# TimingSpace/MVOScaleRecovery

Measured on AMD Instinct MI355X. Metric: frames/sec scale-recovery, KITTI-00 flow (~2k feats/frame), 1/2/4/8 GPU, higher is better.
Workload: dtype f64

## Files before the change

### mvoscalerecovery_amd/csrc/mvosr_kernels.hip

```cpp
#include <hip/hip_runtime.h>
#include <math.h>
#include <stdint.h>
#include <stdlib.h>
#include <string.h>

#include "../../include/mvosr.h"
#include "mvosr_device.hpp"
#include "mvosr_host.hpp"
#include "mvosr_npsum.hpp"

namespace mvosr {

#ifdef MVOSR_STAMPS
#define MVOSR_STAMP(i) do { if (threadIdx.x == 0 && stamps) stamps[i] = __builtin_amdgcn_s_memtime(); } while (0)
#define MVOSR_STAMP_DECL unsigned long long stamps[12] = {0,0,0,0,0,0,0,0,0,0,0,0};
#define MVOSR_STAMP_ARG , unsigned long long *stamps = nullptr
#define MVOSR_STAMP_PASS , stamps
#define MVOSR_RSTAMP(i) do { if (stamps) stamps[i] = __builtin_amdgcn_s_memtime(); } while (0)
#else
#define MVOSR_RSTAMP(i) do {} while (0)
#define MVOSR_STAMP(i) do {} while (0)
#define MVOSR_STAMP_DECL
#define MVOSR_STAMP_ARG
#define MVOSR_STAMP_PASS
// ... 567 lines not shown
            if (base + k * B + tid < t2_count) mark_triangle(base / B + k, tc.q[k].a, tc.q[k].b, tc.q[k].c);
        }
        if (more) tc = tn;
    }
    bad |= bad_in;
    int sn = singular | (near << 16);
    block_sum4i<WAVES>(npitch, ntv, sn, bad, s.red + R_SEL_CNT * 2 * WAVES);
    singular = sn & 0xFFFF;
    r.near = sn >> 16;
    MVOSR_STAMP(5);
    r.height_level = MODE == MODE_HOT ? hl / 3.0 : hl;
    r.n_steep = (int)hcnt;
    r.n_pitch = npitch; r.n_tri_valid = ntv; r.singular = singular; r.bad = bad;
    return r;
}

struct RoadResult {
    double height;
    int status;
    int n_sel, n_kept, n_modes, mode_left, mode_right;
    double mean, std, skew, median;
};

__device__ __forceinline__ bool dropped_by_single(double y, int bin, const Bits192 &single, int first_single) {
    bool d = false;
#pragma unroll
    for (int dk = -1; dk <= 1; ++dk) {
        const int k = bin + dk;
        const bool is_single = (k >= 0) && (k < kBins) && single.test_lane(max(k, 0));
        const double r = bin_edge(k + 1);
        const double lo = r - 0.1;
        const bool in = (k == first_single) ? (y >= lo && y <= r) : (y > lo && y <= r);
        d |= is_single && in;
    }
    return d;
}

#ifdef MVOSR_ROAD_EXACT_COUNT
__device__ unsigned long long g_road_exact_count[3];
#endif
constexpr int kRoadRC = 20;
constexpr int kRoadSub = 4;
constexpr int kRoadWaves = 4;
constexpr int kTrash = 175;
constexpr int kStPending = -1;
constexpr int kStRedo = -2;
static_assert(kStRedo == MVOSR_ST_REDO, "include/mvosr.h");
constexpr int kMaxVoteRows = 32765;

struct RoadArgs {
    mvosr_params P;
    const int64_t *off;
    const int32_t *cnt;
    const double *y;
    double *scratch;
    const double *height_level;
    mvosr_outputs o;
    int64_t first_frame, n_frames;
    int pending_only;
    int32_t *level_redo;
    const int32_t *list;
    int wide;
    const uint8_t *listed_mask = nullptr;
};

__device__ __forceinline__ int bin_of_table(double y, const double2 *edges) {
    if (!(y >= 0.0 && y <= bin_edge(kBins))) return -1;
    int k = min((int)(y * 10.0), kBins - 1);
    const double2 e = edges[k];
    k += (k < kBins - 1 && y >= e.y) ? 1 : 0;
    k -= (y < e.x) ? 1 : 0;
    return k;
}

template <int RC, int WW = 1>
__device__ __forceinline__ RoadResult road_wave(int *hist, int *comb, uint8_t *nearflag, const double2 *edges,
                                                const double *yv_all, double *scratch,
                                                int Mall, double height_level, const mvosr_params &P, int32_t *g_hist, bool exact_stats,
                                                int part_lo, int part_hi, double *part, int *np_stack MVOSR_STAMP_ARG) {
    static_assert(RC <= 32 && kRoadSub == 4, "32-bit row masks; one int4 per bin");
    const int lane = lane_id();
    RoadResult R;
    R.height = nan(""); R.status = MVOSR_ST_MODE; R.n_sel = Mall; R.n_kept = 0; R.n_modes = 0; R.mode_left = -1; R.mode_right = -1;
    R.mean = R.std = R.skew = R.median = nan("");
    if (Mall == 0) { R.status = MVOSR_ST_NO_FLAT; return R; }
    const double *yv = yv_all + (part_hi > part_lo ? part_lo : 0);
    const int M = part_hi - part_lo;
    if (WW == 1 || wave_id() == 0) {
        int4 z; z.x = z.y = z.z = z.w = 0;
#pragma unroll
        for (int c = 0; c < 3; ++c) { const int b = lane + 64 * c; if (b < 176) reinterpret_cast<int4 *>(hist)[b] = z; }
    }
    if constexpr (WW > 1) __syncthreads();
    const double y0 = yv_all[0];
    const double sh = (y0 - y0 == 0.0) ? y0 : 0.0;
    int *hsub = hist + (lane & (kRoadSub - 1));

    const int nfull = M / kWave;
// ... 3 lines not shown
    unsigned pk[(RC + 3) / 4];
    constexpr int kG = 4;
#pragma unroll
    for (int k0 = 0; k0 < RC; k0 += kG) {
        double yg[kG];
#pragma unroll
        for (int j = 0; j < kG && k0 + j < RC; ++j) yg[j] = yv[max(min((k0 + j) * kWave + lane, M - 1), 0)];
#pragma unroll
        for (int j = 0; j < kG && k0 + j < RC; ++j) {
            const int k = k0 + j;
            const double y = yg[j];
            const bool vk = (valid >> k) & 1u;
            const bool inr = vk && (y >= 0.0) && (y <= bin_edge(kBins));
            const int g = inr ? min((int)(y * 10.0), kBins - 1) : 0;
            const double2 e = edges[g];
            int bin = g + ((g < kBins - 1 && y >= e.y) ? 1 : 0) - ((y < e.x) ? 1 : 0);
            bin = inr ? bin : kTrash;
            atomicAdd(&hsub[4 * bin], 1);
            const double d = vk ? y - sh : 0.0;
            s1 += d;
            s2 = __builtin_fma(d, d, s2);
            pk[k >> 2] = (k & 3) ? (pk[k >> 2] | ((unsigned)bin << (8 * (k & 3)))) : (unsigned)bin;
        }
        __builtin_amdgcn_sched_barrier(0);
    }
    constexpr int kLongUnroll = 2;
    for (int i0 = RC * kWave + lane; i0 < M; i0 += kLongUnroll * kWave) {
        double yl[kLongUnroll];
#pragma unroll
        for (int j = 0; j < kLongUnroll; ++j) yl[j] = yv[max(min(i0 + j * kWave, M - 1), 0)];
#pragma unroll
        for (int j = 0; j < kLongUnroll; ++j) {
            if (i0 + j * kWave >= M) continue;
            const int bin = bin_of_table(yl[j], edges);
            if (bin >= 0) atomicAdd(&hsub[4 * bin], 1);
            const double d = yl[j] - sh;
            s1 += d;
            s2 = __builtin_fma(d, d, s2);
        }
    }
    MVOSR_RSTAMP(2);
    if constexpr (WW > 1) __syncthreads();
    int hraw[3], hz[3];
    Bits192 single, modes, mins;
    int mx = 0, mn = 0x7fffffff;
#pragma unroll
    for (int c = 0; c < 3; ++c) {
        const int b = lane + 64 * c;
        int h = 0;
        if (b < kBins) { const int4 q = reinterpret_cast<const int4 *>(hist)[b]; h = (q.x + q.y) + (q.z + q.w); }
        if (b < 176) comb[b] = h;
        hraw[c] = h;
        hz[c] = (hraw[c] == 1) ? 0 : hraw[c];
        single.w[c] = __ballot(b < kBins && hraw[c] == 1);
        mx = max(mx, hz[c]);
        if (b < kBins) mn = min(mn, hz[c]);
    }
    mx = wave_max(mx);
    mn = wave_min(mn);
    if (g_hist && (WW == 1 || wave_id() == 0)) {
#pragma unroll
        for (int c = 0; c < 3; ++c) { const int b = lane + 64 * c; if (b < kBins) { g_hist[b] = hraw[c]; g_hist[kBins + b] = hz[c]; } }
    }
    MVOSR_RSTAMP(3);
    const int first_single = single.lowest_from(0);
    Bits192 near;
    near.w[0] = single.w[0] | (single.w[0] << 1) | (single.w[0] >> 1) | (single.w[1] << 63);
    near.w[1] = single.w[1] | (single.w[1] << 1) | (single.w[1] >> 1) | (single.w[0] >> 63) | (single.w[2] << 63);
    near.w[2] = single.w[2] | (single.w[2] << 1) | (single.w[2] >> 1) | (single.w[1] >> 63);
#pragma unroll
    for (int c = 0; c < 3; ++c) { const int b = lane + 64 * c; if (b < 176) nearflag[b] = (b < kBins) ? (uint8_t)((near.w[c] >> lane) & 1ull) : 0; }
    const bool have_modes = mx > P.mode_min;

    double t1 = 0.0, t2 = 0.0;
    int nd = 0;
    {
        unsigned sus = 0u;
#pragma unroll
        for (int k = 0; k < RC; ++k) sus |= (nearflag[(pk[k >> 2] >> (8 * (k & 3))) & 0xFFu] ? 1u : 0u) << k;
        while (sus) {
            const int k = __ffs(sus) - 1;
            sus &= sus - 1u;
            const double y = yv[k * kWave + lane];
            if (dropped_by_single(y, bin_of_table(y, edges), single, first_single)) {
                const double d = y - sh;
                t1 += d;
                t2 = __builtin_fma(d, d, t2);
                ++nd;
            }
        }
    }
    for (int i0 = RC * kWave + lane; i0 < M; i0 += kLongUnroll * kWave) {
        double yl[kLongUnroll];
#pragma unroll
        for (int j = 0; j < kLongUnroll; ++j) yl[j] = yv[max(min(i0 + j * kWave, M - 1), 0)];
#pragma unroll
        for (int j = 0; j < kLongUnroll; ++j) {
            if (i0 + j * kWave >= M) continue;
            const double y = yl[j];
            const int bin = bin_of_table(y, edges);
            if (bin >= 0 && nearflag[bin] && dropped_by_single(y, bin, single, first_single)) {
                const double d = y - sh;
                t1 += d;
                t2 = __builtin_fma(d, d, t2);
                ++nd;
            }
        }
    }
    double S1 = wave_sum(s1 - t1), S2 = wave_sum(s2 - t2), Q = wave_sum(s2);
    nd = wave_sum(nd);
    if constexpr (WW > 1) {
        if (lane == 0) { part[4 * wave_id()] = S1; part[4 * wave_id() + 1] = S2; part[4 * wave_id() + 2] = Q; part[4 * wave_id() + 3] = (double)nd; }
        __syncthreads();
        S1 = 0.0; S2 = 0.0; Q = 0.0;
        double ndd = 0.0;
#pragma unroll
        for (int i = 0; i < WW; ++i) { S1 += part[4 * i]; S2 += part[4 * i + 1]; Q += part[4 * i + 2]; ndd += part[4 * i + 3]; }
        nd = (int)ndd;
    }
    MVOSR_RSTAMP(4);
    const int nkept = Mall - nd;
    const double cntd = (double)nkept;
    R.n_kept = nkept;

    auto pack_kept = [&]() {
        int nlist = 0;
#pragma unroll 1
        for (int i0 = 0; i0 < Mall; i0 += kWave) {
            const int i = i0 + lane;
            bool keep = false;
            double y = 0.0;
            if (i < Mall) {
                y = yv_all[i];
                const int bin = bin_of_table(y, edges);
                keep = !(bin >= 0 && nearflag[bin] && dropped_by_single(y, bin, single, first_single));
            }
            const unsigned long long m = __ballot(keep);
            if (keep) scratch[nlist + __popcll(m & ((1ull << lane) - 1ull))] = y;
            nlist += __popcll(m);
        }
        return nlist;
    };

    if (!have_modes) {
        if constexpr (WW > 1) { if (wave_id() != 0) return R; }
        if (nkept == 0) { R.height = height_level; R.status = MVOSR_ST_LEVEL; return R; }
        pack_kept();
        __threadfence_block();
        const int klo = (nkept - 1) >> 1, khi = nkept >> 1;
        double mlo = 0.0, mhi = 0.0;
        int flo = 0, fhi = 0;
        for (int i = lane; i < nkept; i += kWave) {
            const double yi = scratch[i];
            int rank = 0;
            for (int j = 0; j < nkept; ++j) {
                const double yj = scratch[j];
                rank += (yj < yi) || (yj == yi && j < i);
            }
            if (rank == klo) { mlo = yi; flo = 1; }
            if (rank == khi) { mhi = yi; fhi = 1; }
        }
        const unsigned long long blo = __ballot(flo), bhi = __ballot(fhi);
        mlo = readlane_d(mlo, (int)__ffsll((long long)blo) - 1);
        mhi = readlane_d(mhi, (int)__ffsll((long long)bhi) - 1);
        R.median = (klo == khi) ? mlo : (mlo + mhi) / 2.0;
        R.height = R.median; R.status = MVOSR_ST_MEDIAN;
        return R;
    }
    if constexpr (WW > 1) { if (wave_id() != 0) return R; }
// ... 32 lines not shown
    const double right = bin_edge(ir + 1);
    const double m1 = S1 / cntd;
    const double mean = sh + m1;
    const double var = S2 / cntd - m1 * m1;
    double mean_o = mean;
    double sd = sqrt(var);
    {
        const double thr = fabs(P.skew_threshold);
        const double N = (double)Mall;
        const double g = 0x1p-52 * (2.0 * (double)((Mall + kWave - 1) / kWave) + 64.0 + N / (double)kNpBufSize);
        const double a2 = Q / cntd, r = sqrt(a2), rho = sqrt(N / cntd), Mg = fabs(sh) + r;
        const double rms = sqrt(mean * mean + var);
        const double margin = fabs((mean - mode / 10.0) - P.skew_threshold * sd);
        const double bound_two_pass = 1e-11 * (rms + sd) + 1e-22 * rms * rms / sd;
        const double bound = bound_two_pass
                           + g * ((Mg + rho * r) + fabs(mode / 10.0) + (1.0 + thr) * sd + (1.0 + thr) * (a2 * (6.0 + 2.0 * rho) + g * Mg * Mg) / sd);
#ifdef MVOSR_ROAD_EXACT_COUNT
        if (lane == 0) {
            atomicAdd(&g_road_exact_count[0], 1ull);
            if (!(margin > bound_two_pass)) atomicAdd(&g_road_exact_count[1], 1ull);
            if (!(margin > bound)) atomicAdd(&g_road_exact_count[2], 1ull);
        }
#endif
        if (!(margin > bound) || exact_stats) {
            const int nl = pack_kept();
            __threadfence_block();
            mean_o = np_pairwise_sum_cold(scratch, nl, 0.0, 0, np_stack) / (double)nl;
            sd = sqrt(np_pairwise_sum_cold(scratch, nl, mean_o, 1, np_stack) / (double)nl);
        }
    }
    const double skew = (mean_o - mode / 10.0) / sd;
    R.mean = mean_o; R.std = sd; R.skew = skew;
    if (skew > P.skew_threshold) { R.height = right; R.status = MVOSR_ST_RIGHT; }
    else { R.height = mode / 10.0; R.status = MVOSR_ST_MODE; }
    return R;
}

constexpr int kRoadOcc = 6;
template <bool LIST, int WW = 1>
__global__ __launch_bounds__(kRoadWaves *kWave, (LIST ? 1 : kRoadOcc)) void road_model_kernel(const RoadArgs a) {
    static_assert(kRoadRC >= 16 && kRoadRC <= 32, "the row masks are 32 bits");
    static_assert(WW == 1 || (WW == kRoadWaves && !LIST), "wide variant: the whole workgroup on one frame");
    __shared__ __attribute__((aligned(16))) int hist_all[kRoadWaves][kRoadSub * 176];
    __shared__ int comb_all[kRoadWaves][176];
    __shared__ uint8_t near_all[kRoadWaves][176];
    __shared__ double2 edges[kBins + 1];
    __shared__ double part[4 * kRoadWaves];
    __shared__ __attribute__((aligned(8))) int np_stack_all[kRoadWaves][kNpStackInts];
    for (int k = threadIdx.x; k < kBins; k += kRoadWaves * kWave) { double2 e; e.x = bin_edge(k); e.y = bin_edge(k + 1); edges[k] = e; }
    __syncthreads();
    const int64_t slot = WW > 1 ? (int64_t)blockIdx.x : (int64_t)blockIdx.x * kRoadWaves + wave_id();
    auto one_frame = [&](const int64_t f) {
    if (a.pending_only && a.o.status[f] != kStPending) return;
    MVOSR_STAMP_DECL
    MVOSR_RSTAMP(0);
    const int M = a.cnt[f];
    const int64_t off = a.off[f];
    const double hl = a.height_level ? a.height_level[f] : nan("");
    MVOSR_RSTAMP(1);
    int *h0 = hist_all[WW > 1 ? 0 : wave_id()];
    int32_t *gh = a.o.hist ? a.o.hist + f * 2 * kBins : nullptr;
    const bool ex = a.o.stats != nullptr;
    int lo = 0, hi = M;
    if constexpr (WW > 1) {
        const int q = ((M + WW * kWave - 1) / (WW * kWave)) * kWave;
        lo = min(M, wave_id() * q);
        hi = min(M, lo + q);
    }
    const int Mp = hi - lo;
#define MVOSR_ROAD_CALL(RC_) road_wave<RC_, WW>(h0, comb_all[wave_id()], near_all[wave_id()], edges, a.y + off, a.scratch + off, M, hl, a.P, gh, ex, lo, hi, part, np_stack_all[wave_id()] MVOSR_STAMP_PASS)
    const RoadResult R = (Mp <= 4 * kWave) ? MVOSR_ROAD_CALL(4)
                       : (Mp <= 8 * kWave) ? MVOSR_ROAD_CALL(8)
                       : (Mp <= 12 * kWave) ? MVOSR_ROAD_CALL(12)
                       : (Mp <= 16 * kWave) ? MVOSR_ROAD_CALL(16)
                                            : MVOSR_ROAD_CALL(kRoadRC);
#undef MVOSR_ROAD_CALL
    MVOSR_RSTAMP(6);
#ifdef MVOSR_STAMPS
    if (lane_id() == 0 && a.o.hist) { unsigned long long *d = reinterpret_cast<unsigned long long *>(a.o.hist + f * 2 * kBins) + 16; for (int i = 0; i < 8; ++i) d[i] = stamps[i]; }
#endif
    if (WW > 1 && wave_id() != 0) return;
    if (R.status == MVOSR_ST_LEVEL && a.level_redo) {
        if (lane_id() == 0) {
            if (!(a.listed_mask && a.listed_mask[f])) a.level_redo[1 + atomicAdd(a.level_redo, 1)] = (int32_t)f;
            a.o.status[f] = kStRedo;
        }
        return;
    }
    if (lane_id() == 0) {
        double height = nan(""), raw = nan("");
        if (R.status == MVOSR_ST_NO_FLAT) raw = a.P.absolute_reference / hl;
        else if (R.status <= MVOSR_ST_LEVEL) { height = R.height; raw = a.P.absolute_reference / height; }
        a.o.raw_scale[f] = raw; a.o.height[f] = height; a.o.status[f] = R.status;
        if (!a.pending_only && a.o.height_level) a.o.height_level[f] = hl;
        if (a.o.counts) {
            int32_t *c = a.o.counts + f * MVOSR_N_COUNTS;
            if (!a.pending_only) { c[MVOSR_CNT_VALID] = M; c[MVOSR_CNT_TRI_PITCH] = 0; c[MVOSR_CNT_TRI_VALID] = 0; }
            c[MVOSR_CNT_SELECTED] = R.n_sel; c[MVOSR_CNT_KEPT] = R.n_kept; c[MVOSR_CNT_MODES] = R.n_modes;
            c[MVOSR_CNT_MODE_LEFT] = R.mode_left; c[MVOSR_CNT_MODE_RIGHT] = R.mode_right;
        }
        if (a.o.stats) { double *st = a.o.stats + 4 * f; st[0] = R.mean; st[1] = R.std; st[2] = R.skew; st[3] = R.median; }
    }
    };
    if constexpr (LIST) {
        const int64_t n_todo = (int64_t)a.list[0];
        for (int64_t it = slot; it < n_todo; it += (int64_t)gridDim.x * kRoadWaves) one_frame((int64_t)a.list[1 + it]);
    } else {
        if (slot < a.n_frames) one_frame(a.first_frame + slot);
    }
}

struct KArgs {
    mvosr_params P;
    mvosr_batch b;
    mvosr_outputs o;
    PitchTest pt;
    int64_t first_frame;
    const double *height_level_in;
    int32_t *redo;
    int redo_pass;
    double *ysel;
    int32_t *nsel;
    const int32_t *cls_list;
    const int32_t *cls_cnt;
};

__device__ __forceinline__ void write_counts(const KArgs &a, int64_t f, int nvalid, int npitch, int ntv, const RoadResult &R) {
    if (!a.o.counts) return;
    int32_t *c = a.o.counts + f * MVOSR_N_COUNTS;
// ... 1042 lines not shown
    if (b->max_feat > variant_capacity(waves, sc))
        return set_error(MVOSR_ERR_TOO_LARGE, "%d features exceed what %d wavefronts per frame handle (%d)", b->max_feat, waves,
                         variant_capacity(waves, sc));
    if ((int64_t)2 * b->max_feat > (int64_t)64 * kWave * waves)
        return set_error(MVOSR_ERR_TOO_LARGE, "%d features give more triangles than %d wavefronts sweep", b->max_feat, waves);
    return MVOSR_OK;
}

__global__ __launch_bounds__(256) void append_mask_kernel(const uint8_t *mask, const int32_t *status, int64_t first, int64_t n, int32_t *redo) {
    const int64_t k = (int64_t)blockIdx.x * blockDim.x + threadIdx.x;
    if (k >= n) return;
    const int64_t f = first + k;
    if (mask[f] && (!status || status[f] == kStPending)) redo[1 + atomicAdd(redo, 1)] = (int32_t)f;
}
static int launch_append_mask(mvosr_ctx *ctx, const KArgs &ka, int64_t nl, bool check_status) {
    if (!ka.b.exact_mask) return MVOSR_OK;
    hipLaunchKernelGGL(append_mask_kernel, dim3((unsigned)((nl + 255) / 256)), dim3(256), 0, ctx_stream(ctx), ka.b.exact_mask,
                       check_status ? ka.o.status : (const int32_t *)nullptr, ka.first_frame, nl, ka.redo);
    return check_launch("append_mask_kernel");
}

constexpr int kRedoGrid = 512;
constexpr int kModeExactList = 3;
static inline KArgs &kargs_of(KArgs &a) { return a; }
static inline KArgs &kargs_of(DenseArgs &a) { return a.k; }

static thread_local bool g_hot_only = false;

template <class Args>
static int launch_modes(mvosr_ctx *ctx, void (*k_hot)(const Args), void (*k_exact)(const Args), void (*k_full)(const Args),
                        Args args, int64_t nl, int threads, size_t lds, int mode, const char *name, size_t lds_hot = 0,
                        int threads_hot = 0) {
    int rc;
    if (lds_hot == 0) lds_hot = lds;
    if (threads_hot == 0) threads_hot = threads;
    kargs_of(args).redo_pass = 0;
    if (mode == MODE_FULL) {
        if ((rc = prepare_kernel(k_full, lds))) return rc;
        hipLaunchKernelGGL(k_full, dim3((unsigned)nl), dim3(threads), lds, ctx_stream(ctx), args);
        return check_launch(name);
    }
    if ((rc = prepare_kernel(k_exact, lds))) return rc;
    if (mode == kModeExactList) {
        kargs_of(args).redo_pass = 1;
        const unsigned grid = (unsigned)(nl < (int64_t)kRedoGrid ? nl : (int64_t)kRedoGrid);
        hipLaunchKernelGGL(k_exact, dim3(grid), dim3(threads), lds, ctx_stream(ctx), args);
        return check_launch(name);
    }
    if (mode == MODE_EXACT) {
        hipLaunchKernelGGL(k_exact, dim3((unsigned)nl), dim3(threads), lds, ctx_stream(ctx), args);
        return check_launch(name);
    }
    if ((rc = prepare_kernel(k_hot, lds_hot))) return rc;
    const hipError_t e = hipMemsetAsync(kargs_of(args).redo, 0, sizeof(int32_t), ctx_stream(ctx));
    if (e != hipSuccess) return set_hip_error("hipMemsetAsync(redo list)", e);
    hipLaunchKernelGGL(k_hot, dim3((unsigned)nl), dim3(threads_hot), lds_hot, ctx_stream(ctx), args);
    if ((rc = check_launch(name))) return rc;
    if (!g_hot_only && (rc = launch_append_mask(ctx, kargs_of(args), nl, true))) return rc;
    return MVOSR_OK;
}

template <int WAVES, int SC>
static int launch_scale(mvosr_ctx *ctx, const KArgs &ka, int64_t nl, int mode) {
    const size_t lds = lds_plan(ka.b.max_feat, WAVES).total;
    int rc = check_fit(&ka.b, WAVES, SC, lds);
    if (rc) return rc;
    return launch_modes<KArgs>(ctx, scale_frames_kernel<WAVES, SC, MODE_HOT>, scale_frames_kernel<WAVES, SC, MODE_EXACT>,
                               scale_frames_kernel<WAVES, SC, MODE_FULL>, ka, nl, WAVES * kWave, lds, mode, "scale_frames_kernel");
}

template <int WAVES, int SC>
static int launch_vote(mvosr_ctx *ctx, const KArgs &ka, int64_t nl) {
    const size_t lds = lds_plan(ka.b.max_feat, WAVES).total;
    int rc = check_fit(&ka.b, WAVES, SC, lds);
    if (rc) return rc;
    if ((rc = prepare_kernel(outlier_vote_kernel<WAVES, SC>, lds))) return rc;
    hipLaunchKernelGGL((outlier_vote_kernel<WAVES, SC>), dim3((unsigned)nl), dim3(WAVES * kWave), lds, ctx_stream(ctx), ka);
    return check_launch("outlier_vote_kernel");
// ... 22 lines not shown
    }
    if (vote_only) {
        if ((rc = prepare_kernel(outlier_vote_dense_kernel<DW>, lds))) return rc;
        hipLaunchKernelGGL((outlier_vote_dense_kernel<DW>), dim3((unsigned)nl), dim3(DW * kWave), lds, ctx_stream(ctx), da);
        return check_launch("outlier_vote_dense_kernel");
    }
    if (tiled)
        return launch_modes<DenseArgs>(ctx, scale_frames_tiled_kernel<kTiledWaves>, scale_frames_dense_feat_kernel<DW, MODE_EXACT>,
                                       scale_frames_dense_feat_kernel<DW, MODE_FULL>, da, nl, DW * kWave, lds, mode,
                                       "scale_frames_tiled_kernel", tiled_plan(ka.b.max_feat, kTiledWaves).total, kTiledWaves * kWave);
    if (ka.b.tri2_ids == MVOSR_TRI2_FEATURES)
        return launch_modes<DenseArgs>(ctx, scale_frames_dense_feat_kernel<DW, MODE_HOT>, scale_frames_dense_feat_kernel<DW, MODE_EXACT>,
                                       scale_frames_dense_feat_kernel<DW, MODE_FULL>, da, nl, DW * kWave, lds, mode,
                                       "scale_frames_dense_feat_kernel");
    return launch_modes<DenseArgs>(ctx, scale_frames_dense_kernel<DW, MODE_HOT>, scale_frames_dense_kernel<DW, MODE_EXACT>,
                                   scale_frames_dense_kernel<DW, MODE_FULL>, da, nl, DW * kWave, lds, mode, "scale_frames_dense_kernel");
}

static int launch_scale_dense(mvosr_ctx *ctx, const KArgs &ka, int64_t nl, int mode, bool vote_only) {
    if (ka.b.max_feat > 65535) return set_error(MVOSR_ERR_TOO_LARGE, "more than 65535 features per frame");
    return launch_scale_dense_w<kDenseWaves>(ctx, ka, nl, mode, vote_only);
}

static int launch_road(mvosr_ctx *ctx, const RoadArgs &ra, hipStream_t stream) {
    if (ra.n_frames <= 0) return MVOSR_OK;
    if (ra.wide && !ra.list) {
        hipLaunchKernelGGL((road_model_kernel<false, kRoadWaves>), dim3((unsigned)ra.n_frames), dim3(kRoadWaves * kWave), 0, stream, ra);
        return check_launch("road_model_kernel (wide)");
    }
    const unsigned blocks = ra.list ? 64u : (unsigned)((ra.n_frames + kRoadWaves - 1) / kRoadWaves);
    if (ra.list) hipLaunchKernelGGL(road_model_kernel<true>, dim3(blocks), dim3(kRoadWaves * kWave), 0, stream, ra);
    else hipLaunchKernelGGL(road_model_kernel<false>, dim3(blocks), dim3(kRoadWaves * kWave), 0, stream, ra);
    return check_launch("road_model_kernel");
}

#define MVOSR_DISPATCH(FN, ...)                                                             \
    do {                                                                                    \
        const int n_ = ka.b.max_feat;                                                       \
        switch (waves) {                                                                    \
            case 1: return FN<1, 8>(__VA_ARGS__);                                           \
            case 4: return (n_ <= variant_capacity(4, 4)) ? FN<4, 4>(__VA_ARGS__) : FN<4, 8>(__VA_ARGS__);     \
            case 16: return (n_ <= variant_capacity(16, 4)) ? FN<16, 4>(__VA_ARGS__) : FN<16, 8>(__VA_ARGS__); \
            default: return (n_ <= variant_capacity(8, 4)) ? FN<8, 4>(__VA_ARGS__) : FN<8, 8>(__VA_ARGS__);    \
        }                                                                                   \
    } while (0)

static int dispatch_scale(mvosr_ctx *ctx, const KArgs &ka, int waves, int64_t nl, int mode) { MVOSR_DISPATCH(launch_scale, ctx, ka, nl, mode); }
static int dispatch_vote(mvosr_ctx *ctx, const KArgs &ka, int waves, int64_t nl) { MVOSR_DISPATCH(launch_vote, ctx, ka, nl); }

typedef void (*scale_kernel_fn)(const KArgs);
static scale_kernel_fn hot_list_kernel(int waves, int n) {
    switch (waves) {
        case 1: return scale_frames_kernel<1, 8, MODE_HOT, true>;
        case 4: return (n <= variant_capacity(4, 4)) ? scale_frames_kernel<4, 4, MODE_HOT, true> : scale_frames_kernel<4, 8, MODE_HOT, true>;
// ... 14 lines not shown
    scale_kernel_fn fn[3];
    int waves[3];
    size_t lds[3];
    KArgs kc[3];
    for (int c = 0; c < 3; ++c) {
        kc[c] = ka;
        kc[c].b.max_feat = thr[c] < ka.b.max_feat ? thr[c] : ka.b.max_feat;
        const int n = kc[c].b.max_feat;
        waves[c] = pick_waves(0, n);
        lds[c] = lds_plan(n, waves[c]).total;
        fn[c] = hot_list_kernel(waves[c], n);
        const int sc = (n <= variant_capacity(waves[c], 4) && waves[c] != 1) ? 4 : 8;
        if ((rc = check_fit(&kc[c].b, waves[c], sc, lds[c]))) return rc;
        if ((rc = prepare_kernel(fn[c], lds[c]))) return rc;
        int64_t bound = hinted && (int64_t)ka.b.size_hint[c] < nl ? (int64_t)ka.b.size_hint[c] : nl;
        if ((c > 0 && thr[c - 1] >= ka.b.max_feat) || ka.b.min_feat > thr[c]) bound = 0;
        ca.grid[c] = (int)(bound < 0 ? 0 : bound);
        kc[c].cls_list = ca.lists + c * ca.stride;
        kc[c].cls_cnt = hdr + c;
        kc[c].redo_pass = 0;
    }
    if ((e = hipMemsetAsync(hdr, 0, kClassHeader * sizeof(int32_t), ctx_stream(ctx))) != hipSuccess)
        return set_hip_error("hipMemsetAsync(class lists)", e);
    if ((e = hipMemsetAsync(ka.redo, 0, sizeof(int32_t), ctx_stream(ctx))) != hipSuccess)
        return set_hip_error("hipMemsetAsync(redo list)", e);
    const int cb = kClassifyWaves * kWave;
    hipLaunchKernelGGL(classify_frames_kernel, dim3((unsigned)((nl + cb - 1) / cb)), dim3(cb), 0, ctx_stream(ctx), ca);
    if ((rc = check_launch("classify_frames_kernel"))) return rc;
    for (int c = 2; c >= 0; --c) {
        if (ca.grid[c] == 0) continue;
        hipLaunchKernelGGL(fn[c], dim3((unsigned)ca.grid[c]), dim3(waves[c] * kWave), lds[c], ctx_stream(ctx), kc[c]);
        if ((rc = check_launch("scale_frames_kernel (size class)"))) return rc;
    }
    return MVOSR_OK;
}

void set_max_dynamic_lds(int bytes) { g_max_dyn_lds = bytes; }

}

using namespace mvosr;

extern "C" {

void mvosr_default_params(mvosr_params *p, double absolute_reference) {
    if (!p) return;
    const double pitch = -0.5 * 3.141592653589793 / 180.0;
    p->cos_pitch = cos(pitch);
// ... 46 lines not shown
    ra.P = *p; ra.off = b->feat_off; ra.cnt = ka.nsel; ra.y = ka.ysel; ra.scratch = ka.ysel;
    ra.height_level = o->height_level; ra.o = *o; ra.pending_only = 1; ra.level_redo = nullptr; ra.list = nullptr; ra.wide = 0;
    ka.first_frame = first_frame;
    if (b->tri2_ids != MVOSR_TRI2_SURVIVORS && b->tri2_ids != MVOSR_TRI2_FEATURES)
        return set_error(MVOSR_ERR_ARG, "scale_batch: batch.tri2_ids must be MVOSR_TRI2_SURVIVORS or MVOSR_TRI2_FEATURES");
    if (b->tri2_ids == MVOSR_TRI2_FEATURES && !(waves_per_frame == 0 || waves_per_frame == 16))
        return set_error(MVOSR_ERR_ARG, "scale_batch: feature-numbered tri2 runs the gather variant (waves_per_frame 0 or 16)");
    const bool dense = (waves_per_frame == 0 || waves_per_frame == 16) &&
                       (b->max_feat > lds_capacity_features() || b->tri2_ids == MVOSR_TRI2_FEATURES);
    hipEvent_t *pev = (ctx->prof_on && ctx->prof_calls < kProfRing) ? ctx->prof_ev[ctx->prof_calls] : nullptr;
    hipError_t ee = hipSuccess;
    if (pev && (ee = hipEventRecord(pev[0], ctx_stream(ctx))) != hipSuccess) return set_hip_error("hipEventRecord(profile)", ee);
    const bool by_class = mode == MODE_HOT && !dense && waves_per_frame == 0 && n_launch >= kClassMinFrames &&
                          b->max_feat > kClassThr0 &&
                          (b->min_feat <= 0 || pick_waves(0, b->min_feat) != waves);
    const bool standin = b->standin_u != nullptr;
    if (standin) {
        if (!b->standin_keep || !b->standin_rows || !b->standin_cnt || !b->standin_status || !b->tri2_cnt || b->tri2_ids != MVOSR_TRI2_SURVIVORS)
            return set_error(MVOSR_ERR_ARG, "scale_batch: stand-in rows need standin_keep/_rows/_cnt/_status, tri2_cnt and survivor-numbered rows");
        if (dense) return set_error(MVOSR_ERR_TOO_LARGE, "scale_batch: stand-in rows are for frames that fit the LDS-resident kernels");
        if (!(want_masked || mode == MODE_HOT))
            return set_error(MVOSR_ERR_ARG, "scale_batch: stand-in rows need the HOT mode (no stage outputs, no EXACT-for-all)");
    }
    auto road = [&]() {
#ifdef MVOSR_STAMPS
        return MVOSR_OK;
#else
        return launch_road(ctx, ra, ctx_stream(ctx));
#endif
    };
    auto standin_rows = [&](const int32_t *list) {
        return qh_rows_for_list(ctx, b->n_frames, b->feat_off, b->feat_cnt, b->standin_u, b->v, b->standin_keep, b->max_feat, b->tri2_off,
                                b->standin_rows, b->standin_cnt, b->standin_status, list);
    };
    if (want_masked) {
        if (!b->exact_mask) return set_error(MVOSR_ERR_ARG, "scale_batch: MVOSR_WAVES_EXACT_MASKED without batch.exact_mask");
        const hipError_t e0 = hipMemsetAsync(ka.redo, 0, sizeof(int32_t), ctx_stream(ctx));
        if (e0 != hipSuccess) return set_hip_error("hipMemsetAsync(redo list)", e0);
        if ((rc = launch_append_mask(ctx, ka, n_launch, false))) return rc;
        if (standin && (rc = standin_rows(ka.redo))) return rc;
        if ((rc = dense ? launch_scale_dense(ctx, ka, n_launch, kModeExactList, false) : dispatch_scale(ctx, ka, waves, n_launch, kModeExactList))) return rc;
        ra.first_frame = first_frame; ra.n_frames = n_launch; ra.list = ka.redo;
        ra.wide = dense ? 1 : 0;
        return road();
    }
    if (by_class) {
        if ((rc = launch_scale_classes(ctx, ka, n_launch))) return rc;
        if (!hot_only && (rc = launch_append_mask(ctx, ka, n_launch, true))) return rc;
    } else {
        g_hot_only = hot_only;
        rc = dense ? launch_scale_dense(ctx, ka, n_launch, mode, false) : dispatch_scale(ctx, ka, waves, n_launch, mode);
        g_hot_only = false;
        if (rc) return rc;
    }
    if (pev && (ee = hipEventRecord(pev[1], ctx_stream(ctx))) != hipSuccess) return set_hip_error("hipEventRecord(profile)", ee);
    ra.first_frame = first_frame; ra.n_frames = n_launch;
    ra.wide = dense ? 1 : 0;
    if (mode == MODE_HOT) {
        ra.level_redo = ka.redo;
        ra.listed_mask = hot_only ? nullptr : b->exact_mask;
        if ((rc = road())) return rc;
        ra.listed_mask = nullptr;
        if (hot_only) return MVOSR_OK;
        if (standin && (rc = standin_rows(ka.redo))) return rc;
        if ((rc = dense ? launch_scale_dense(ctx, ka, n_launch, kModeExactList, false) : dispatch_scale(ctx, ka, waves, n_launch, kModeExactList))) return rc;
        ra.level_redo = nullptr; ra.list = ka.redo;
        if ((rc = road())) return rc;
    } else if ((rc = road())) {
        return rc;
    }
    if (pev) {
        if ((ee = hipEventRecord(pev[2], ctx_stream(ctx))) != hipSuccess) return set_hip_error("hipEventRecord(profile)", ee);
        ctx->prof_calls++;
    }
    return MVOSR_OK;
}

int mvosr_batch_size_hint(const int32_t *feat_cnt_host, int64_t n_frames, mvosr_batch *b) {
    if (!b || n_frames < 0 || (n_frames > 0 && !feat_cnt_host)) return set_error(MVOSR_ERR_ARG, "batch_size_hint: null argument");
    int64_t cnt[3] = {0, 0, 0};
    int32_t lo = 0, hi = 0;
    for (int64_t f = 0; f < n_frames; ++f) {
        const int32_t n = feat_cnt_host[f];
        if (n < 0) return set_error(MVOSR_ERR_ARG, "batch_size_hint: negative feature count");
        if (f == 0 || n < lo) lo = n;
        if (f == 0 || n > hi) hi = n;
        ++cnt[size_class_of(n)];
    }
    b->max_feat = hi;
    b->min_feat = lo;
    for (int c = 0; c < 3; ++c) b->size_hint[c] = (int32_t)(cnt[c] > 0x7fffffff ? 0x7fffffff : cnt[c]);
    b->size_hint[3] = kClassHintMagic;
// ... 11 lines not shown
    KArgs ka;
    ka.P = *p; ka.b = *b; ka.o = *o; ka.pt = make_pitch_test(p->pitch_threshold_deg);
    ka.first_frame = 0; ka.height_level_in = nullptr; ka.ysel = nullptr; ka.nsel = nullptr; ka.redo = nullptr; ka.redo_pass = 0;
    ka.cls_list = nullptr; ka.cls_cnt = nullptr;
    if ((waves_per_frame == 0 || waves_per_frame == 16) && b->max_feat > lds_capacity_features()) {
        if (b->total_feat <= 0) return set_error(MVOSR_ERR_ARG, "outlier_vote: batch.total_feat not set");
        return launch_scale_dense(ctx, ka, b->n_frames, MODE_HOT, true);
    }
    return dispatch_vote(ctx, ka, pick_waves(waves_per_frame, b->max_feat), b->n_frames);
}

int mvosr_road_model_batch(mvosr_ctx *ctx, const mvosr_params *p, const mvosr_batch *b, const double *height_level_in,
                           const mvosr_outputs *o, int waves_per_frame) {
    (void)waves_per_frame;
    int rc = check_common(ctx, p, b, o);
    if (rc) return rc;
    if (!b->y) return set_error(MVOSR_ERR_ARG, "road_model: y plane required");
    if (!o->raw_scale || !o->height || !o->status) return set_error(MVOSR_ERR_ARG, "road_model: raw_scale/height/status required");
    if (b->n_frames == 0) return MVOSR_OK;
    if (b->total_feat <= 0) return set_error(MVOSR_ERR_ARG, "road_model: batch.total_feat (length of the y plane) not set");
    if ((rc = ctx_activate(ctx))) return rc;
    RoadArgs ra;
    double *scratch = nullptr;
    int32_t *unused = nullptr;
    if ((rc = ctx_workspace(ctx, b->n_frames, b->total_feat, &scratch, &unused))) return rc;
    ra.P = *p; ra.off = b->feat_off; ra.cnt = b->feat_cnt; ra.y = b->y; ra.scratch = scratch;
    ra.height_level = height_level_in; ra.o = *o;
    ra.first_frame = 0; ra.n_frames = b->n_frames; ra.pending_only = 0; ra.level_redo = nullptr; ra.list = nullptr;
    ra.wide = b->max_feat > 4 * kRoadRC * kWave ? 1 : 0;
    return launch_road(ctx, ra, ctx_stream(ctx));
}

static int launch_window_median(mvosr_ctx *ctx, const double *raw, int64_t n, int n_blocks, int64_t stride, int window,
                                const double *queue_in, int n_queue, double *out) {
    if (!ctx || (n > 0 && (!raw || !out))) return set_error(MVOSR_ERR_ARG, "window_median: null argument");
    if (window < 1 || window > kMaxWindow) return set_error(MVOSR_ERR_ARG, "window_median: window must be in 1..%d", kMaxWindow);
    if (n_queue < 0 || n_queue > window || (n_queue > 0 && !queue_in)) return set_error(MVOSR_ERR_ARG, "window_median: bad carried-in queue");
    if (n_blocks < 1) return set_error(MVOSR_ERR_ARG, "window_median: n_blocks < 1");
    if (n <= 0) return MVOSR_OK;
    MedianArgs ma;
    ma.raw = raw; ma.out = out; ma.n = n; ma.window = window; ma.n_queue = n_queue;
    ma.n_blocks = n_blocks; ma.base_len = n / n_blocks; ma.extra = n % n_blocks; ma.stride = stride;
    if (n_blocks > 1 && stride < ma.base_len + (ma.extra ? 1 : 0)) return set_error(MVOSR_ERR_ARG, "window_median: block stride shorter than a block");
    int rc = ctx_activate(ctx);
    if (rc) return rc;
    for (int i = 0; i < kMaxWindow; ++i) ma.queue[i] = (i < n_queue) ? queue_in[i] : 0.0;
    hipLaunchKernelGGL(window_median_kernel, dim3((unsigned)((n + 255) / 256)), dim3(256), 0, ctx_stream(ctx), ma);
    return check_launch("window_median_kernel");
}

int mvosr_window_median(mvosr_ctx *ctx, const double *raw, int64_t n, int window, const double *queue_in, int n_queue,
                        double *out) {
    return launch_window_median(ctx, raw, n, 1, 0, window, queue_in, n_queue, out);
// ... 21 lines not shown
```

Baseline: 26.30 million.

## Split road model into lean hot kernel with cold-frame fallback list

Adds a HOT variant of the road model kernel that handles only short frames on the fast path, with no histogram or stats output, no long tail loop and no exact-stats fallback. Frames that need the slow path are appended to a cold list, which a second list-driven launch then processes. The intent is to cut register pressure and raise occupancy (launch bounds 7) for the common case. Per-frame scalars are moved to readfirstlane and the single-bin bitmask is passed as three words. The cost is an extra kernel launch, a larger memset, and atomics on the cold list.

```diff
diff --git a/mvoscalerecovery_amd/csrc/mvosr_kernels.hip b/mvoscalerecovery_amd/csrc/mvosr_kernels.hip
--- a/mvoscalerecovery_amd/csrc/mvosr_kernels.hip
+++ b/mvoscalerecovery_amd/csrc/mvosr_kernels.hip
@@ -613,12 +613,14 @@
     double mean, std, skew, median;
 };
 
-__device__ __forceinline__ bool dropped_by_single(double y, int bin, const Bits192 &single, int first_single) {
+__device__ __forceinline__ bool dropped_by_single(double y, int bin, unsigned long long s0, unsigned long long s1, unsigned long long s2,
+                                                  int first_single) {
     bool d = false;
 #pragma unroll
     for (int dk = -1; dk <= 1; ++dk) {
         const int k = bin + dk;
-        const bool is_single = (k >= 0) && (k < kBins) && single.test_lane(max(k, 0));
+        const int kk = max(k, 0);
+        const bool is_single = (k >= 0) && (k < kBins) && (((kk < 64 ? s0 : (kk < 128 ? s1 : s2)) >> (kk & 63)) & 1ull);
         const double r = bin_edge(k + 1);
         const double lo = r - 0.1;
         const bool in = (k == first_single) ? (y >= lo && y <= r) : (y > lo && y <= r);
@@ -631,11 +633,13 @@
 __device__ unsigned long long g_road_exact_count[3];
 #endif
 constexpr int kRoadRC = 20;
+constexpr int kRoadRCHot = 24;
 constexpr int kRoadSub = 4;
 constexpr int kRoadWaves = 4;
 constexpr int kTrash = 175;
 constexpr int kStPending = -1;
 constexpr int kStRedo = -2;
+constexpr int kStCold = -3;
 static_assert(kStRedo == MVOSR_ST_REDO, "include/mvosr.h");
 constexpr int kMaxVoteRows = 32765;
 
@@ -653,6 +657,7 @@
     const int32_t *list;
     int wide;
     const uint8_t *listed_mask = nullptr;
+    int32_t *cold = nullptr;
 };
 
 __device__ __forceinline__ int bin_of_table(double y, const double2 *edges) {
@@ -664,7 +669,7 @@
     return k;
 }
 
-template <int RC, int WW = 1>
+template <int RC, int WW = 1, bool HOT = false>
 __device__ __forceinline__ RoadResult road_wave(int *hist, int *comb, uint8_t *nearflag, const double2 *edges,
                                                 const double *yv_all, double *scratch,
                                                 int Mall, double height_level, const mvosr_params &P, int32_t *g_hist, bool exact_stats,
@@ -714,9 +719,13 @@
             s2 = __builtin_fma(d, d, s2);
             pk[k >> 2] = (k & 3) ? (pk[k >> 2] | ((unsigned)bin << (8 * (k & 3)))) : (unsigned)bin;
         }
+        asm volatile("" : "+v"(s1), "+v"(s2));
+        static_assert(kG == 4, "one word of pk per group");
+        asm volatile("" : "+v"(pk[k0 >> 2]));
         __builtin_amdgcn_sched_barrier(0);
     }
     constexpr int kLongUnroll = 2;
+    if constexpr (!HOT) {
     for (int i0 = RC * kWave + lane; i0 < M; i0 += kLongUnroll * kWave) {
         double yl[kLongUnroll];
 #pragma unroll
@@ -730,6 +739,7 @@
             s1 += d;
             s2 = __builtin_fma(d, d, s2);
         }
+    }
     }
     MVOSR_RSTAMP(2);
     if constexpr (WW > 1) __syncthreads();
@@ -750,12 +760,13 @@
     }
     mx = wave_max(mx);
     mn = wave_min(mn);
-    if (g_hist && (WW == 1 || wave_id() == 0)) {
+    if (!HOT && g_hist && (WW == 1 || wave_id() == 0)) {
 #pragma unroll
         for (int c = 0; c < 3; ++c) { const int b = lane + 64 * c; if (b < kBins) { g_hist[b] = hraw[c]; g_hist[kBins + b] = hz[c]; } }
     }
     MVOSR_RSTAMP(3);
     const int first_single = single.lowest_from(0);
+    const unsigned long long sg0 = single.w[0], sg1 = single.w[1], sg2 = single.w[2];
     Bits192 near;
     near.w[0] = single.w[0] | (single.w[0] << 1) | (single.w[0] >> 1) | (single.w[1] << 63);
     near.w[1] = single.w[1] | (single.w[1] << 1) | (single.w[1] >> 1) | (single.w[0] >> 63) | (single.w[2] << 63);
@@ -774,7 +785,7 @@
             const int k = __ffs(sus) - 1;
             sus &= sus - 1u;
             const double y = yv[k * kWave + lane];
-            if (dropped_by_single(y, bin_of_table(y, edges), single, first_single)) {
+            if (dropped_by_single(y, bin_of_table(y, edges), sg0, sg1, sg2, first_single)) {
                 const double d = y - sh;
                 t1 += d;
                 t2 = __builtin_fma(d, d, t2);
@@ -782,6 +793,7 @@
             }
         }
     }
+    if constexpr (!HOT) {
     for (int i0 = RC * kWave + lane; i0 < M; i0 += kLongUnroll * kWave) {
         double yl[kLongUnroll];
 #pragma unroll
@@ -791,13 +803,14 @@
             if (i0 + j * kWave >= M) continue;
             const double y = yl[j];
             const int bin = bin_of_table(y, edges);
-            if (bin >= 0 && nearflag[bin] && dropped_by_single(y, bin, single, first_single)) {
+            if (bin >= 0 && nearflag[bin] && dropped_by_single(y, bin, sg0, sg1, sg2, first_single)) {
                 const double d = y - sh;
                 t1 += d;
                 t2 = __builtin_fma(d, d, t2);
                 ++nd;
             }
         }
+    }
     }
     double S1 = wave_sum(s1 - t1), S2 = wave_sum(s2 - t2), Q = wave_sum(s2);
     nd = wave_sum(nd);
@@ -825,7 +838,7 @@
             if (i < Mall) {
                 y = yv_all[i];
                 const int bin = bin_of_table(y, edges);
-                keep = !(bin >= 0 && nearflag[bin] && dropped_by_single(y, bin, single, first_single));
+                keep = !(bin >= 0 && nearflag[bin] && dropped_by_single(y, bin, sg0, sg1, sg2, first_single));
             }
             const unsigned long long m = __ballot(keep);
             if (keep) scratch[nlist + __popcll(m & ((1ull << lane) - 1ull))] = y;
@@ -837,6 +850,7 @@
     if (!have_modes) {
         if constexpr (WW > 1) { if (wave_id() != 0) return R; }
         if (nkept == 0) { R.height = height_level; R.status = MVOSR_ST_LEVEL; return R; }
+        if constexpr (HOT) { R.status = kStCold; return R; }
         pack_kept();
         __threadfence_block();
         const int klo = (nkept - 1) >> 1, khi = nkept >> 1;
@@ -915,7 +929,9 @@
             if (!(margin > bound)) atomicAdd(&g_road_exact_count[2], 1ull);
         }
 #endif
-        if (!(margin > bound) || exact_stats) {
+        if constexpr (HOT) {
+            if (!(margin > bound)) { R.status = kStCold; return R; }
+        } else if (!(margin > bound) || exact_stats) {
             const int nl = pack_kept();
             __threadfence_block();
             mean_o = np_pairwise_sum_cold(scratch, nl, 0.0, 0, np_stack) / (double)nl;
@@ -930,10 +946,12 @@
 }
 
 constexpr int kRoadOcc = 6;
-template <bool LIST, int WW = 1>
-__global__ __launch_bounds__(kRoadWaves *kWave, (LIST ? 1 : kRoadOcc)) void road_model_kernel(const RoadArgs a) {
-    static_assert(kRoadRC >= 16 && kRoadRC <= 32, "the row masks are 32 bits");
+constexpr int kRoadOccHot = 7;
+template <bool LIST, int WW = 1, bool HOT = false>
+__global__ __launch_bounds__(kRoadWaves *kWave, (LIST ? 1 : HOT ? kRoadOccHot : kRoadOcc)) void road_model_kernel(const RoadArgs a) {
+    static_assert(kRoadRC >= 16 && kRoadRC <= 32 && kRoadRCHot >= 16 && kRoadRCHot <= 32, "the row masks are 32 bits");
     static_assert(WW == 1 || (WW == kRoadWaves && !LIST), "wide variant: the whole workgroup on one frame");
+    static_assert(!HOT || (!LIST && WW == 1), "the lean variant: one wavefront per frame, no list");
     __shared__ __attribute__((aligned(16))) int hist_all[kRoadWaves][kRoadSub * 176];
     __shared__ int comb_all[kRoadWaves][176];
     __shared__ uint8_t near_all[kRoadWaves][176];
@@ -944,16 +962,19 @@
     __syncthreads();
     const int64_t slot = WW > 1 ? (int64_t)blockIdx.x : (int64_t)blockIdx.x * kRoadWaves + wave_id();
     auto one_frame = [&](const int64_t f) {
-    if (a.pending_only && a.o.status[f] != kStPending) return;
+    const int st_in = a.pending_only ? __builtin_amdgcn_readfirstlane(a.o.status[f]) : kStPending;
+    const int M = __builtin_amdgcn_readfirstlane(a.cnt[f]);
+    const int64_t off_l = a.off[f];
+    const int64_t off = (int64_t)(((uint64_t)(uint32_t)__builtin_amdgcn_readfirstlane((int)(off_l >> 32)) << 32) |
+                                  (uint64_t)(uint32_t)__builtin_amdgcn_readfirstlane((int)off_l));
+    const double hl = a.height_level ? a.height_level[f] : nan("");
+    if (st_in != kStPending) return;
     MVOSR_STAMP_DECL
     MVOSR_RSTAMP(0);
-    const int M = a.cnt[f];
-    const int64_t off = a.off[f];
-    const double hl = a.height_level ? a.height_level[f] : nan("");
     MVOSR_RSTAMP(1);
     int *h0 = hist_all[WW > 1 ? 0 : wave_id()];
-    int32_t *gh = a.o.hist ? a.o.hist + f * 2 * kBins : nullptr;
-    const bool ex = a.o.stats != nullptr;
+    int32_t *gh = (!HOT && a.o.hist) ? a.o.hist + f * 2 * kBins : nullptr;
+    const bool ex = !HOT && a.o.stats != nullptr;
     int lo = 0, hi = M;
     if constexpr (WW > 1) {
         const int q = ((M + WW * kWave - 1) / (WW * kWave)) * kWave;
@@ -961,12 +982,27 @@
         hi = min(M, lo + q);
     }
     const int Mp = hi - lo;
-#define MVOSR_ROAD_CALL(RC_) road_wave<RC_, WW>(h0, comb_all[wave_id()], near_all[wave_id()], edges, a.y + off, a.scratch + off, M, hl, a.P, gh, ex, lo, hi, part, np_stack_all[wave_id()] MVOSR_STAMP_PASS)
-    const RoadResult R = (Mp <= 4 * kWave) ? MVOSR_ROAD_CALL(4)
-                       : (Mp <= 8 * kWave) ? MVOSR_ROAD_CALL(8)
-                       : (Mp <= 12 * kWave) ? MVOSR_ROAD_CALL(12)
-                       : (Mp <= 16 * kWave) ? MVOSR_ROAD_CALL(16)
-                                            : MVOSR_ROAD_CALL(kRoadRC);
+#define MVOSR_ROAD_CALL(RC_) road_wave<RC_, WW, HOT>(h0, comb_all[wave_id()], near_all[wave_id()], edges, a.y + off, a.scratch + off, M, hl, a.P, gh, ex, lo, hi, part, np_stack_all[wave_id()] MVOSR_STAMP_PASS)
+    RoadResult R;
+    if constexpr (HOT) {
+        if (Mp > kRoadRCHot * kWave) R.status = kStCold;
+        else R = (Mp <= 4 * kWave) ? MVOSR_ROAD_CALL(4)
+               : (Mp <= 8 * kWave) ? MVOSR_ROAD_CALL(8)
+               : (Mp <= 12 * kWave) ? MVOSR_ROAD_CALL(12)
+               : (Mp <= 16 * kWave) ? MVOSR_ROAD_CALL(16)
+               : (Mp <= 20 * kWave) ? MVOSR_ROAD_CALL(20)
+                                    : MVOSR_ROAD_CALL(kRoadRCHot);
+        if (R.status == kStCold) {
+            if (lane_id() == 0 && !(a.listed_mask && a.listed_mask[f])) a.cold[1 + atomicAdd(a.cold, 1)] = (int32_t)f;
+            return;
+        }
+    } else {
+        R = (Mp <= 4 * kWave) ? MVOSR_ROAD_CALL(4)
+          : (Mp <= 8 * kWave) ? MVOSR_ROAD_CALL(8)
+          : (Mp <= 12 * kWave) ? MVOSR_ROAD_CALL(12)
+          : (Mp <= 16 * kWave) ? MVOSR_ROAD_CALL(16)
+                               : MVOSR_ROAD_CALL(kRoadRC);
+    }
 #undef MVOSR_ROAD_CALL
     MVOSR_RSTAMP(6);
 #ifdef MVOSR_STAMPS
@@ -992,12 +1028,15 @@
             c[MVOSR_CNT_SELECTED] = R.n_sel; c[MVOSR_CNT_KEPT] = R.n_kept; c[MVOSR_CNT_MODES] = R.n_modes;
             c[MVOSR_CNT_MODE_LEFT] = R.mode_left; c[MVOSR_CNT_MODE_RIGHT] = R.mode_right;
         }
-        if (a.o.stats) { double *st = a.o.stats + 4 * f; st[0] = R.mean; st[1] = R.std; st[2] = R.skew; st[3] = R.median; }
+        if constexpr (!HOT) {
+            if (a.o.stats) { double *st = a.o.stats + 4 * f; st[0] = R.mean; st[1] = R.std; st[2] = R.skew; st[3] = R.median; }
+        }
     }
     };
     if constexpr (LIST) {
-        const int64_t n_todo = (int64_t)a.list[0];
+        const int64_t n_todo = a.list ? (int64_t)a.list[0] : 0, n_cold = a.cold ? (int64_t)a.cold[0] : 0;
         for (int64_t it = slot; it < n_todo; it += (int64_t)gridDim.x * kRoadWaves) one_frame((int64_t)a.list[1 + it]);
+        for (int64_t it = slot; it < n_cold; it += (int64_t)gridDim.x * kRoadWaves) one_frame((int64_t)a.cold[1 + it]);
     } else {
         if (slot < a.n_frames) one_frame(a.first_frame + slot);
     }
@@ -2086,6 +2125,13 @@
 
 constexpr int kRedoGrid = 512;
 constexpr int kModeExactList = 3;
+
+static inline int32_t *cold_list_of(int32_t *redo, int64_t n_frames) { return redo + 1 + n_frames; }
+static int zero_lists(mvosr_ctx *ctx, int32_t *redo, int64_t n_frames) {
+    const size_t bytes = (((size_t)n_frames + 2) * sizeof(int32_t) + 15) & ~(size_t)15;
+    const hipError_t e = hipMemsetAsync(redo, 0, bytes, ctx_stream(ctx));
+    return e == hipSuccess ? MVOSR_OK : set_hip_error("hipMemsetAsync(redo and cold lists)", e);
+}
 static inline KArgs &kargs_of(KArgs &a) { return a; }
 static inline KArgs &kargs_of(DenseArgs &a) { return a.k; }
 
@@ -2116,8 +2162,7 @@
         return check_launch(name);
     }
     if ((rc = prepare_kernel(k_hot, lds_hot))) return rc;
-    const hipError_t e = hipMemsetAsync(kargs_of(args).redo, 0, sizeof(int32_t), ctx_stream(ctx));
-    if (e != hipSuccess) return set_hip_error("hipMemsetAsync(redo list)", e);
+    if ((rc = zero_lists(ctx, kargs_of(args).redo, kargs_of(args).b.n_frames))) return rc;
     hipLaunchKernelGGL(k_hot, dim3((unsigned)nl), dim3(threads_hot), lds_hot, ctx_stream(ctx), args);
     if ((rc = check_launch(name))) return rc;
     if (!g_hot_only && (rc = launch_append_mask(ctx, kargs_of(args), nl, true))) return rc;
@@ -2186,14 +2231,18 @@
     return launch_scale_dense_w<kDenseWaves>(ctx, ka, nl, mode, vote_only);
 }
 
-static int launch_road(mvosr_ctx *ctx, const RoadArgs &ra, hipStream_t stream) {
+static int launch_road(mvosr_ctx *ctx, const RoadArgs &ra, hipStream_t stream, bool lists = false) {
     if (ra.n_frames <= 0) return MVOSR_OK;
-    if (ra.wide && !ra.list) {
+    if (lists) {
+        hipLaunchKernelGGL(road_model_kernel<true>, dim3(64u), dim3(kRoadWaves * kWave), 0, stream, ra);
+        return check_launch("road_model_kernel (lists)");
+    }
+    if (ra.wide) {
         hipLaunchKernelGGL((road_model_kernel<false, kRoadWaves>), dim3((unsigned)ra.n_frames), dim3(kRoadWaves * kWave), 0, stream, ra);
         return check_launch("road_model_kernel (wide)");
     }
-    const unsigned blocks = ra.list ? 64u : (unsigned)((ra.n_frames + kRoadWaves - 1) / kRoadWaves);
-    if (ra.list) hipLaunchKernelGGL(road_model_kernel<true>, dim3(blocks), dim3(kRoadWaves * kWave), 0, stream, ra);
+    const unsigned blocks = (unsigned)((ra.n_frames + kRoadWaves - 1) / kRoadWaves);
+    if (ra.cold) hipLaunchKernelGGL((road_model_kernel<false, 1, true>), dim3(blocks), dim3(kRoadWaves * kWave), 0, stream, ra);
     else hipLaunchKernelGGL(road_model_kernel<false>, dim3(blocks), dim3(kRoadWaves * kWave), 0, stream, ra);
     return check_launch("road_model_kernel");
 }
@@ -2254,8 +2303,7 @@
     }
     if ((e = hipMemsetAsync(hdr, 0, kClassHeader * sizeof(int32_t), ctx_stream(ctx))) != hipSuccess)
         return set_hip_error("hipMemsetAsync(class lists)", e);
-    if ((e = hipMemsetAsync(ka.redo, 0, sizeof(int32_t), ctx_stream(ctx))) != hipSuccess)
-        return set_hip_error("hipMemsetAsync(redo list)", e);
+    if ((rc = zero_lists(ctx, ka.redo, ka.b.n_frames))) return rc;
     const int cb = kClassifyWaves * kWave;
     hipLaunchKernelGGL(classify_frames_kernel, dim3((unsigned)((nl + cb - 1) / cb)), dim3(cb), 0, ctx_stream(ctx), ca);
     if ((rc = check_launch("classify_frames_kernel"))) return rc;
@@ -2348,11 +2396,11 @@
         if (!(want_masked || mode == MODE_HOT))
             return set_error(MVOSR_ERR_ARG, "scale_batch: stand-in rows need the HOT mode (no stage outputs, no EXACT-for-all)");
     }
-    auto road = [&]() {
+    auto road = [&](bool lists = false) {
 #ifdef MVOSR_STAMPS
         return MVOSR_OK;
 #else
-        return launch_road(ctx, ra, ctx_stream(ctx));
+        return launch_road(ctx, ra, ctx_stream(ctx), lists);
 #endif
     };
     auto standin_rows = [&](const int32_t *list) {
@@ -2367,8 +2415,7 @@
         if (standin && (rc = standin_rows(ka.redo))) return rc;
         if ((rc = dense ? launch_scale_dense(ctx, ka, n_launch, kModeExactList, false) : dispatch_scale(ctx, ka, waves, n_launch, kModeExactList))) return rc;
         ra.first_frame = first_frame; ra.n_frames = n_launch; ra.list = ka.redo;
-        ra.wide = dense ? 1 : 0;
-        return road();
+        return road(true);
     }
     if (by_class) {
         if ((rc = launch_scale_classes(ctx, ka, n_launch))) return rc;
@@ -2382,18 +2429,25 @@
     if (pev && (ee = hipEventRecord(pev[1], ctx_stream(ctx))) != hipSuccess) return set_hip_error("hipEventRecord(profile)", ee);
     ra.first_frame = first_frame; ra.n_frames = n_launch;
     ra.wide = dense ? 1 : 0;
+    const bool lean = !dense && !hot_only && !o->stats && !o->hist;
     if (mode == MODE_HOT) {
         ra.level_redo = ka.redo;
         ra.listed_mask = hot_only ? nullptr : b->exact_mask;
+        ra.cold = lean ? cold_list_of(ka.redo, b->n_frames) : nullptr;
         if ((rc = road())) return rc;
         ra.listed_mask = nullptr;
         if (hot_only) return MVOSR_OK;
         if (standin && (rc = standin_rows(ka.redo))) return rc;
         if ((rc = dense ? launch_scale_dense(ctx, ka, n_launch, kModeExactList, false) : dispatch_scale(ctx, ka, waves, n_launch, kModeExactList))) return rc;
         ra.level_redo = nullptr; ra.list = ka.redo;
+        if ((rc = road(true))) return rc;
+    } else {
+        if (lean) {
+            ra.cold = cold_list_of(ka.redo, b->n_frames);
+            if ((ee = hipMemsetAsync(ra.cold, 0, sizeof(int32_t), ctx_stream(ctx))) != hipSuccess) return set_hip_error("hipMemsetAsync(cold list)", ee);
+        }
         if ((rc = road())) return rc;
-    } else if ((rc = road())) {
-        return rc;
+        if (lean && (rc = road(true))) return rc;
     }
     if (pev) {
         if ((ee = hipEventRecord(pev[2], ctx_stream(ctx))) != hipSuccess) return set_hip_error("hipEventRecord(profile)", ee);
@@ -2451,13 +2505,18 @@
     if ((rc = ctx_activate(ctx))) return rc;
     RoadArgs ra;
     double *scratch = nullptr;
-    int32_t *unused = nullptr;
-    if ((rc = ctx_workspace(ctx, b->n_frames, b->total_feat, &scratch, &unused))) return rc;
+    int32_t *ints = nullptr;
+    if ((rc = ctx_workspace(ctx, b->n_frames, b->total_feat, &scratch, &ints))) return rc;
     ra.P = *p; ra.off = b->feat_off; ra.cnt = b->feat_cnt; ra.y = b->y; ra.scratch = scratch;
     ra.height_level = height_level_in; ra.o = *o;
     ra.first_frame = 0; ra.n_frames = b->n_frames; ra.pending_only = 0; ra.level_redo = nullptr; ra.list = nullptr;
     ra.wide = b->max_feat > 4 * kRoadRC * kWave ? 1 : 0;
-    return launch_road(ctx, ra, ctx_stream(ctx));
+    if (ra.wide || o->stats || o->hist) return launch_road(ctx, ra, ctx_stream(ctx));
+    ra.cold = cold_list_of(ints + b->n_frames, b->n_frames);
+    const hipError_t e = hipMemsetAsync(ra.cold, 0, sizeof(int32_t), ctx_stream(ctx));
+    if (e != hipSuccess) return set_hip_error("hipMemsetAsync(cold list)", e);
+    if ((rc = launch_road(ctx, ra, ctx_stream(ctx)))) return rc;
+    return launch_road(ctx, ra, ctx_stream(ctx), true);
 }
 
 static int launch_window_median(mvosr_ctx *ctx, const double *raw, int64_t n, int n_blocks, int64_t stride, int window,
diff --git a/profiles/road_cold_count.py b/profiles/road_cold_count.py
--- /dev/null
+++ b/profiles/road_cold_count.py
@@ -0,0 +1,50 @@
+#!/usr/bin/env python3
+import ctypes as C
+import os
+import runpy
+import sys
+
+import numpy as np
+
+R = os.path.dirname(os.path.dirname(os.path.abspath(__file__)))
+sys.path.insert(0, R)
+from mvoscalerecovery_amd import _lib
+
+
+class CtxHead(C.Structure):
+    _fields_ = [("device", C.c_int), ("own_stream", C.c_void_p), ("stream", C.c_void_p), ("n_cu", C.c_int),
+                ("max_lds_per_block", C.c_int), ("name", C.c_char * 128), ("ws_ysel", C.c_void_p), ("ws_ysel_len", C.c_size_t),
+                ("ws_nsel", C.c_void_p), ("ws_nsel_len", C.c_size_t)]
+
+
+def report(ctx):
+    head = CtxHead.from_address(ctx.handle.value)
+    if not head.ws_nsel or head.n_cu != ctx.n_cu:
+        return
+    F = int(head.ws_nsel_len)
+    ctx.sync()
+    words = np.empty(2 * (F + 1), dtype=np.int32)
+    _lib.check(ctx.lib.mvosr_memcpy_d2h(ctx.handle, C.c_void_p(words.ctypes.data), C.c_void_p(head.ws_nsel + 4 * F), C.c_size_t(words.nbytes)), "d2h")
+    print("road lists after the last step: frames %d  redo list %d  cold list %d = %.3g of the frames" % (F, words[0], words[F + 1], words[F + 1] / max(F, 1)),
+          file=sys.stderr)
+
+
+created = []
+_init = _lib.Context.__init__
+
+
+def init(self, *a, **k):
+    _init(self, *a, **k)
+    created.append(self)
+
+
+_lib.Context.__init__ = init
+sys.argv = [os.path.join(R, "bench.py"), "--no-cpu-baseline", "--no-e2e"] + sys.argv[1:]
+try:
+    runpy.run_path(sys.argv[0], run_name="__main__")
+except SystemExit as e:
+    if e.code not in (None, 0):
+        raise
+for ctx in created:
+    if getattr(ctx, "handle", None):
+        report(ctx)
```

Result: faster. 26.96 million (median of 6 runs) (+2.5%).
